# openai/ot-gan

Hardware: AMD Instinct MI355X
Metric: OT-GAN train images/sec (CIFAR-10 32x32, bs=256/GPU) (higher is better)
Workload: dtype f32 (Winograd-domain GEMMs on the fp16 matrix pipe with operands split into two scaled fp16 pieces = 22 significand bits, fp32 accumulate; errors at or below the fp32 MFMA chain's)

## Files before the change

### ot-gan_amd/csrc/winograd.hip

```cpp
#ifndef X3_PIECES
#define X3_PIECES 2
#endif
#ifndef WINO_NS
#define WINO_NS wino_p2
#endif
#include "winograd.h"
#include "gemm_x3.h"
#include <type_traits>

#include <stdlib.h>

#include <algorithm>
#include <array>
#include <atomic>
#include <map>
#include <mutex>
#include <vector>

#include "gemm_tile.h"

namespace WINO_NS {

namespace {

using Cfg = GemmCfg<2, 2, 2, 2, 32>;

template <auto Kern>
inline void ensure_lds(size_t bytes) {
  static const bool done = [bytes] {
    hipFuncSetAttribute(reinterpret_cast<const void*>(Kern), hipFuncAttributeMaxDynamicSharedMemorySize,
                        (int)bytes);
    return true;
  }();
  (void)done;
}


constexpr int WA = kWA;
constexpr int WM = kWA - 2;
constexpr int WF = kWF;
static_assert(WA == 6, "the transforms below are written for F(4x4, 3x3)");

typedef double f64x4 __attribute__((ext_vector_type(4)));

__device__ __forceinline__ f32x4 ld4(const float* p) { return *reinterpret_cast<const f32x4*>(p); }
__device__ __forceinline__ void st4(float* p, f32x4 v) { *reinterpret_cast<f32x4*>(p) = v; }

__device__ __forceinline__ float hdr_scale(const u16* P, int f) {
#if X3_PIECES == 2
  return P ? (reinterpret_cast<const float*>(P) - X3_HDR)[16 + f] : 1.f;
#else
  return 1.f;
#endif
}
__device__ __forceinline__ void st_operand(float* F, u16* P, long rows, int ld, int f, long row, int k, f32x4 v, float sc) {
  if (P) {
    const long fs = op_fstride(rows, ld);
#if X3_PIECES == 2
    st_split4h(P, WF * fs, f * fs + op_off(row, k, ld >> 4), v * sc);
#else
    st_split4(P, WF * fs, f * fs + op_off(row, k, ld >> 4), v);
#endif
  } else {
    st4(F + ((long)f * rows + row) * ld + k, v);
  }
}

__device__ __forceinline__ bool op_thread(bool blocked, long rows, int nk4, long& row, int& k4) {
  if (blocked) {
    const int kgroups = (nk4 + 15) >> 4;
    const long b = blockIdx.x;
    k4 = (int)(b % kgroups) * 16 + (threadIdx.x >> 6) * 4 + (threadIdx.x & 3);
    row = (b / kgroups) * 16 + ((threadIdx.x >> 2) & 15);
  } else {
    const long idx = (long)blockIdx.x * 256 + threadIdx.x;
    k4 = (int)(idx % nk4);
    row = idx / nk4;
  }
  return row < rows && k4 < nk4;
}
inline int op_grid(long rows, long nk4) { return (int)(((rows + 15) / 16) * ((nk4 + 15) / 16)); }

__device__ __forceinline__ void bt1(const f32x4 (&x)[WA], f32x4 (&y)[WA]) {
  y[0] = x[0] - 1.5f * x[1] - 2.f * x[2] + 1.5f * x[3] + x[4];
  y[1] = 0.5f * x[2] - x[1] + 2.5f * x[3] + x[4];
  y[2] = x[1] - 2.5f * x[2] + 0.5f * x[3] + x[4];
  y[3] = 2.f * (x[3] - x[1]) - x[2] + x[4];
  y[4] = 0.5f * (x[1] - x[3]) - x[2] + x[4];
  y[5] = x[1] - 1.5f * x[2] - 2.f * x[3] + 1.5f * x[4] + x[5];
}
template <class V>
__device__ __forceinline__ void at1(const V (&x)[WA], V (&y)[WM]) {
  const V s = x[1] + x[2], d = x[1] - x[2];
  y[0] = x[0] + s + x[3] + x[4];
  y[1] = d + 0.5f * x[3] - 2.f * x[4];
  y[2] = s + 0.25f * x[3] + 4.f * x[4];
  y[3] = d + 0.125f * x[3] - 8.f * x[4] + x[5];
}
__device__ __forceinline__ void a1(const f32x4 (&y)[WM], f32x4 (&x)[WA]) {
  x[0] = y[0];
  x[1] = y[0] + y[1] + y[2] + y[3];
  x[2] = y[0] - y[1] + y[2] - y[3];
  x[3] = y[0] + 0.5f * y[1] + 0.25f * y[2] + 0.125f * y[3];
  x[4] = y[0] - 2.f * y[1] + 4.f * y[2] - 8.f * y[3];
  x[5] = y[3];
}
__device__ __forceinline__ void g1(const f64x4 (&g)[3], f64x4 (&u)[WA]) {
  u[0] = g[0];
  u[1] = (g[0] + g[1] + g[2]) * (1.0 / 3.0);
  u[2] = (g[1] - g[0] - g[2]) * (1.0 / 3.0);
  u[3] = (4.0 * g[0] + 2.0 * g[1] + g[2]) * (-4.0 / 15.0);
  u[4] = (g[0] - 2.0 * g[1] + 4.0 * g[2]) * (1.0 / 15.0);
  u[5] = g[2];
}
__device__ __forceinline__ void gt1(const f32x4 (&u)[WA], f32x4 (&g)[3]) {
  const f32x4 a = u[1] * (1.f / 3.f), b = u[2] * (1.f / 3.f), c = u[3] * (-4.f / 15.f), d = u[4] * (1.f / 15.f);
  g[0] = u[0] + a - b + 4.f * c + d;
  g[1] = a + b + 2.f * c - 2.f * d;
  g[2] = a - b + c + 4.f * d + u[5];
}
__device__ __forceinline__ f64x4 to_d(f32x4 v) { return __builtin_convertvector(v, f64x4); }
__device__ __forceinline__ f32x4 to_f(f64x4 v) { return __builtin_convertvector(v, f32x4); }

template <class Emit>
__device__ __forceinline__ void tf_filter(const f32x4 (&g)[3][3], Emit&& emit) {
  f64x4 t[WA][3];
#pragma unroll
  for (int j = 0; j < 3; ++j) {
    const f64x4 col[3] = {to_d(g[0][j]), to_d(g[1][j]), to_d(g[2][j])};
    f64x4 u[WA];
    g1(col, u);
#pragma unroll
    for (int i = 0; i < WA; ++i) t[i][j] = u[i];
  }
#pragma unroll
  for (int i = 0; i < WA; ++i) {
    f64x4 u[WA];
    g1(t[i], u);
#pragma unroll
    for (int j = 0; j < WA; ++j) emit(i * WA + j, to_f(u[j]));
  }
}
template <class Col>
__device__ __forceinline__ void tf_filter_adj(Col&& col, f32x4 (&dg)[3][3]) {
  f32x4 p[3][WA];
#pragma unroll
  for (int j = 0; j < WA; ++j) {
    f32x4 u[WA], g[3];
    col(j, u);
    gt1(u, g);
#pragma unroll
    for (int i = 0; i < 3; ++i) p[i][j] = g[i];
  }
#pragma unroll
  for (int i = 0; i < 3; ++i) gt1(p[i], dg[i]);
}

struct AmaxArgs {
  const float* x;
  long rows, ld;
  int C;
  float* hdr;
  float gain[WA];
  float fold;
  int floor_one;
  int record_only;
  int nrec;
  float* scratch;
  unsigned* counter;
};
constexpr float kGainBt[WA] = {7.f, 5.f, 5.f, 6.f, 3.f, 7.f};
constexpr float kGainG[WA] = {1.f, 1.f, 1.f, 28.f / 15.f, 7.f / 15.f, 1.f};
constexpr float kGainA[WA] = {1.f, 4.f, 4.f, 1.875f, 15.f, 1.f};
constexpr int kAmaxBlocks = 2048, kAmaxSlots = 64;

__device__ __forceinline__ void write_scales(const AmaxArgs& a, float amax, int tid) {
  if (a.record_only == 2) {
    if (tid == 0) {
      unsigned* p = reinterpret_cast<unsigned*>(a.hdr);
      const unsigned b = __float_as_uint(amax) & 0x7fffffffu;
      if (b > *p) *p = b;
    }
    return;
  }
  if (a.record_only) {
    if (tid < kAmaxSub) a.hdr[tid * kAmaxSubStride] = tid == 0 ? amax : 0.f;
    return;
  }
  if (a.floor_one && amax == amax) amax = fmaxf(amax, 1.f);
  if (tid < WF) {
    const int i = tid / WA, j = tid - i * WA;
    const float bound = amax * a.fold * (a.gain[i] * a.gain[j]);
    float sc = 1.f, inv = 1.f;
    if (!(bound <= 3.0e38f)) {
// ... 57 lines not shown
#pragma unroll
    for (int w = 1; w < 4; ++w) r = (r == r && red[w] == red[w]) ? fmaxf(r, red[w]) : __builtin_nanf("");
    return r;
  };
  m = block_max(m);
  if (tid == 0) {
    __hip_atomic_store(&a.scratch[blockIdx.x], m, __ATOMIC_RELAXED, __HIP_MEMORY_SCOPE_AGENT);
    asm volatile("s_waitcnt vmcnt(0)" ::: "memory");
    last = __hip_atomic_fetch_add(a.counter, 1u, __ATOMIC_RELAXED, __HIP_MEMORY_SCOPE_AGENT) == gridDim.x - 1;
  }
  __syncthreads();
  if (!last) return;
  float r = 0.f;
  for (int i = tid; i < (int)gridDim.x; i += 256) {
    const float w = __hip_atomic_load(&a.scratch[i], __ATOMIC_RELAXED, __HIP_MEMORY_SCOPE_AGENT);
    r = (r == r && w == w) ? fmaxf(r, w) : __builtin_nanf("");
  }
  const float amax = block_max(r);
  write_scales(a, amax, tid);
  if (tid == 0) *a.counter = 0;
}
__global__ __launch_bounds__(64) void scales_from_amax_kernel(AmaxArgs a) { write_scales(a, amax_records_value(a.x, a.nrec), threadIdx.x); }

struct View {
  const float* p;
  long sn, sh, sw;
};
struct WView {
  float* p;
  long sn, sh, sw;
};

struct ScaleSrc {
  const float* rec;
  int nrec;
  float gain[WA];
  float fold;
  int floor_one;
};
__device__ __forceinline__ void producer_scale_table(const ScaleSrc& ss, u16* P, float* s_sc) {
#if X3_PIECES == 2
  if (P) {
    const int tid = threadIdx.x;
    if (tid < WF) {
      float* hdr = reinterpret_cast<float*>(P) - X3_HDR;
      float sc;
      if (ss.rec) {
        float amax = amax_records_value(ss.rec, ss.nrec);
        if (ss.floor_one && amax == amax) amax = fmaxf(amax, 1.f);
        const int i = tid / WA, j = tid - i * WA;
        const float bound = amax * ss.fold * (ss.gain[i] * ss.gain[j]);
        float inv = 1.f;
        sc = 1.f;
        if (!(bound <= 3.0e38f)) {
          sc = inv = __builtin_nanf("");
        } else if (bound > 0.f) {
          const int e = x3_scale_exp(amax * ss.fold, ss.gain[i], ss.gain[j]);
          sc = __builtin_ldexpf(1.f, 14 - e);
          inv = __builtin_ldexpf(1.f, e - 14);
        }
        if (blockIdx.x == 0 && blockIdx.y == 0 && blockIdx.z == 0) {
          hdr[16 + tid] = sc;
          hdr[64 + tid] = inv;
          if (tid == 0) hdr[0] = amax;
        }
      } else {
        sc = hdr[16 + tid];
      }
      s_sc[tid] = sc;
    }
    __syncthreads();
  }
#endif
}
struct InArgs {
  ScaleSrc ss;
  View v[4];
  int coff[4];
  int H, W, TH, TW, C;
  long T;
  int ldv;
  float* V;
  int s2_skip;
  u16* P;
  int up;
  int Cpad;
};
template <int ACT>
__device__ __forceinline__ f32x4 wino_act(f32x4 v) {
#pragma unroll
  for (int j = 0; j < 4; ++j) {
    if (ACT == 1) v[j] = fmaxf(v[j], 0.f);
    if (ACT == 2) v[j] = v[j] > 0.f ? v[j] : expm1f(v[j]);
  }
  return v;
}
template <int ACT, bool DOUBLED>
__global__ __launch_bounds__(256) void wino_input_kernel(InArgs a) {
  __shared__ float s_sc[WF];
  producer_scale_table(a.ss, a.P, s_sc);
  long t;
  int k4;
  if (!op_thread(a.P != nullptr, a.T, (a.Cpad > a.C ? a.Cpad : a.C) >> 2, t, k4)) return;
  const int c = k4 * 4;
  const int tb = (int)(t % a.TW), ta = (int)((t / a.TW) % a.TH);
  const long n = t / ((long)a.TW * a.TH);
  const int cls = blockIdx.z;
  const View v = a.v[cls];
  const int pass = DOUBLED ? (int)blockIdx.y : 0;
  const f32x4 zero = {0.f, 0.f, 0.f, 0.f};
  if (c >= a.C) {
    for (int f = 0; f < WF; ++f) st_operand(a.V, a.P, a.T, a.ldv, f, t, c, zero, 1.f);
    return;
  }
  f32x4 T[WA][WA];
#pragma unroll
  for (int j = 0; j < WA; ++j) {
    const int q = WM * tb - 1 + j;
    f32x4 col[WA], o[WA];
#pragma unroll
    for (int i = 0; i < WA; ++i) {
      const int r = WM * ta - 1 + i;
      const bool ok = (unsigned)r < (unsigned)a.H && (unsigned)q < (unsigned)a.W;
      f32x4 e = ok ? ld4(v.p + n * v.sn + (r >> a.up) * v.sh + (q >> a.up) * v.sw + c) : zero;
      if (ACT != 0 || DOUBLED) e = wino_act<ACT>(pass ? -e : e);
      col[i] = e;
    }
    bt1(col, o);
#pragma unroll
    for (int i = 0; i < WA; ++i) T[i][j] = o[i];
  }
  const int k0 = a.coff[cls] + c + (pass ? a.C : 0);
#pragma unroll
  for (int i = 0; i < WA; ++i) {
    f32x4 o[WA];
    bt1(T[i], o);
#pragma unroll
    for (int j = 0; j < WA; ++j)
      if (a.s2_skip < 0 || s2_present(cls, i * WA + j, a.s2_skip)) st_operand(a.V, a.P, a.T, a.ldv, i * WA + j, t, k0, o[j], s_sc[i * WA + j]);
  }
}

struct OutArgs {
  WView v[4];
  int coff[4];
  int TH, TW, C;
  long T;
  int ldm;
  const float* Mh;
  const float* bias;
  int accumulate;
  float* amax;
  WView gv[4];
};
__global__ __launch_bounds__(256) void wino_output_kernel(OutArgs a) {
  const int c4n = a.C >> 2;
  const long idx = (long)blockIdx.x * 256 + threadIdx.x;
  if (idx >= a.T * c4n) return;
  unsigned mb = 0u;
  const int c = (int)(idx % c4n) * 4;
  const long t = idx / c4n;
  const int tb = (int)(t % a.TW), ta = (int)((t / a.TW) % a.TH);
  const long n = t / ((long)a.TW * a.TH);
  const WView v = a.v[blockIdx.z];
  const float* in = a.Mh + t * a.ldm + a.coff[blockIdx.z] + c;
  const long fs = a.T * a.ldm;
  f32x4 S[WM][WA];
#pragma unroll
  for (int j = 0; j < WA; ++j) {
    f32x4 col[WA], o[WM];
#pragma unroll
    for (int i = 0; i < WA; ++i) col[i] = ld4(in + (i * WA + j) * fs);
    at1(col, o);
#pragma unroll
    for (int i = 0; i < WM; ++i) S[i][j] = o[i];
  }
  f32x4 b = {0.f, 0.f, 0.f, 0.f};
  if (a.bias) b = ld4(a.bias + c);
#pragma unroll
  for (int i = 0; i < WM; ++i) {
    f32x4 y[WM];
    at1(S[i], y);
#pragma unroll
    for (int j = 0; j < WM; ++j) {
      float* dst = v.p + n * v.sn + (WM * ta + i) * v.sh + (WM * tb + j) * v.sw + c;
      f32x4 o = y[j] + b;
      if (a.accumulate) o += ld4(dst);
      mb = amax_bits4(o, mb);
      st4(dst, o);
    }
  }
  if (a.amax) amax_commit(a.amax, mb);
}

__device__ __forceinline__ float wino_sigmoid(float x) { return 1.f / (1.f + expf(-x)); }
__global__ __launch_bounds__(256) void wino_output_glu_kernel(OutArgs a) {
  const int ch = a.C >> 1, c4n = ch >> 2;
  const long idx = (long)blockIdx.x * 256 + threadIdx.x;
  if (idx >= a.T * c4n) return;
  unsigned mb = 0u;
  const int c = (int)(idx % c4n) * 4;
  const long t = idx / c4n;
  const int tb = (int)(t % a.TW), ta = (int)((t / a.TW) % a.TH);
  const long n = t / ((long)a.TW * a.TH);
  const WView v = a.v[blockIdx.z], gv = a.gv[blockIdx.z];
  const long fs = a.T * a.ldm;
#pragma unroll
  for (int half = 0; half < 2; ++half) {
    const int cc = c + half * ch;
    const float* in = a.Mh + t * a.ldm + a.coff[blockIdx.z] + cc;
    f32x4 S[WM][WA];
#pragma unroll
    for (int j = 0; j < WA; ++j) {
      f32x4 col[WA], o[WM];
#pragma unroll
      for (int i = 0; i < WA; ++i) col[i] = ld4(in + (i * WA + j) * fs);
      at1(col, o);
#pragma unroll
      for (int i = 0; i < WM; ++i) S[i][j] = o[i];
    }
    f32x4 b = {0.f, 0.f, 0.f, 0.f};
    if (a.bias) b = ld4(a.bias + cc);
#pragma unroll
    for (int i = 0; i < WM; ++i) {
      f32x4 y[WM];
      at1(S[i], y);
#pragma unroll
      for (int j = 0; j < WM; ++j) {
        float* dst = v.p + n * v.sn + (WM * ta + i) * v.sh + (WM * tb + j) * v.sw + c;
        const f32x4 o = y[j] + b;
        st4(dst + half * ch, o);
        if (half) {
          const f32x4 val = ld4(dst);
          f32x4 gl;
#pragma unroll
          for (int k = 0; k < 4; ++k) gl[k] = val[k] * wino_sigmoid(o[k]);
          mb = amax_bits4(gl, mb);
          st4(gv.p + n * gv.sn + (WM * ta + i) * gv.sh + (WM * tb + j) * gv.sw + c, gl);
        }
      }
    }
  }
  if (a.amax) amax_commit(a.amax, mb);
}

__global__ __launch_bounds__(256) void op_zero_cols_kernel(u16* P, long rows, int ld, int k0, int k1) {
  long row;
  int k4;
  if (!op_thread(true, rows, (k1 - k0) >> 2, row, k4)) return;
  const f32x4 z = {0.f, 0.f, 0.f, 0.f};
  for (int f = 0; f < WF; ++f) st_operand(nullptr, P, rows, ld, f, row, k0 + 4 * k4, z, 1.f);
}

__global__ __launch_bounds__(256) void wino_outadj_kernel(InArgs a) {
  __shared__ float s_sc[WF];
  producer_scale_table(a.ss, a.P, s_sc);
  long t;
  int k4;
  if (!op_thread(a.P != nullptr, a.T, a.C >> 2, t, k4)) return;
  const int c = k4 * 4;
  const int tb = (int)(t % a.TW), ta = (int)((t / a.TW) % a.TH);
  const long n = t / ((long)a.TW * a.TH);
  const View v = a.v[blockIdx.z];
  f32x4 u[WA][WM];
#pragma unroll
  for (int j = 0; j < WM; ++j) {
    f32x4 col[WM], o[WA];
#pragma unroll
    for (int i = 0; i < WM; ++i) col[i] = ld4(v.p + n * v.sn + (WM * ta + i) * v.sh + (WM * tb + j) * v.sw + c);
    a1(col, o);
#pragma unroll
    for (int i = 0; i < WA; ++i) u[i][j] = o[i];
  }
#pragma unroll
  for (int i = 0; i < WA; ++i) {
    f32x4 o[WA];
    a1(u[i], o);
#pragma unroll
    for (int j = 0; j < WA; ++j) st_operand(a.V, a.P, a.T, a.ldv, i * WA + j, t, a.coff[blockIdx.z] + c, o[j], s_sc[i * WA + j]);
  }
}

__global__ __launch_bounds__(256) void wino_filter_fwd_kernel(const float* __restrict__ weffT, long cls_stride,
                                                            int Cin, int Cout, float* __restrict__ U, u16* P) {
  const long rows = 4L * Cout;
  long row;
  int k4;
  if (!op_thread(P != nullptr, rows, Cin >> 2, row, k4)) return;
  const int ci = k4 * 4;
  const int cls = (int)(row / Cout), co = (int)(row % Cout);
  const float* src = weffT + cls * cls_stride + (long)co * 9 * Cin + ci;
  f32x4 g[3][3];
#pragma unroll
  for (int i = 0; i < 3; ++i)
#pragma unroll
    for (int j = 0; j < 3; ++j) g[i][j] = ld4(src + (long)(i * 3 + j) * Cin);
  tf_filter(g, [&](int f, f32x4 v) { st_operand(U, P, rows, Cin, f, row, ci, v, hdr_scale(P, f)); });
}

__global__ __launch_bounds__(256) void wino_filter_bwd_kernel(const float* __restrict__ weff, long cls_stride,
                                                            int Cin, int Cout, float* __restrict__ U, u16* P) {
  const int c4n = Cout >> 2;
  long row;
  int k4;
  if (!op_thread(P != nullptr, Cin, 4 * c4n, row, k4)) return;
  const int ci = (int)row, cls = k4 / c4n, co = (k4 % c4n) * 4;
  const float* src = weff + cls * cls_stride + (long)ci * Cout + co;
  f32x4 g[3][3];
#pragma unroll
  for (int i = 0; i < 3; ++i)
#pragma unroll
    for (int j = 0; j < 3; ++j) g[i][j] = ld4(src + (long)((2 - i) * 3 + (2 - j)) * Cin * Cout);
  tf_filter(g, [&](int f, f32x4 v) { st_operand(U, P, Cin, 4 * Cout, f, ci, cls * Cout + co, v, hdr_scale(P, f)); });
}

__device__ __forceinline__ int fold5_tap(int p, int k) { return p ? (k + 1) >> 1 : k >> 1; }

__global__ __launch_bounds__(256) void wino_filter_fwd_unfolded_kernel(const float* __restrict__ wT, int Cin, int Cout,
                                                                     float* __restrict__ U, u16* P) {
  const long rows = 4L * Cout;
  long row;
  int k4;
  if (!op_thread(P != nullptr, rows, Cin >> 2, row, k4)) return;
  const int ci = k4 * 4;
  const int cls = (int)(row / Cout), co = (int)(row % Cout);
  const int ph = cls >> 1, pw = cls & 1;
  const float* src = wT + (long)co * 25 * Cin + ci;
  const f32x4 zero = {0.f, 0.f, 0.f, 0.f};
  f32x4 g[3][3];
#pragma unroll
  for (int i = 0; i < 3; ++i)
#pragma unroll
    for (int j = 0; j < 3; ++j) g[i][j] = zero;
#pragma unroll
  for (int kh = 0; kh < 5; ++kh)
#pragma unroll
    for (int kw = 0; kw < 5; ++kw) {
      const f32x4 v = ld4(src + (long)(kh * 5 + kw) * Cin);
#pragma unroll
      for (int i = 0; i < 3; ++i)
#pragma unroll
        for (int j = 0; j < 3; ++j)
          if (fold5_tap(ph, kh) == i && fold5_tap(pw, kw) == j) g[i][j] += v;
    }
  tf_filter(g, [&](int f, f32x4 v) { st_operand(U, P, rows, Cin, f, row, ci, v, hdr_scale(P, f)); });
}

__global__ __launch_bounds__(256) void wino_filter_bwd_unfolded_kernel(const float* __restrict__ w, int Cin, int Cout,
                                                                     float* __restrict__ U, u16* P) {
  const int c4n = Cout >> 2;
  long row;
  int k4;
  if (!op_thread(P != nullptr, Cin, 4 * c4n, row, k4)) return;
  const int ci = (int)row, cls = k4 / c4n, co = (k4 % c4n) * 4;
  const int ph = cls >> 1, pw = cls & 1;
  const float* src = w + (long)ci * Cout + co;
  const f32x4 zero = {0.f, 0.f, 0.f, 0.f};
  f32x4 g[3][3];
#pragma unroll
  for (int i = 0; i < 3; ++i)
#pragma unroll
    for (int j = 0; j < 3; ++j) g[i][j] = zero;
#pragma unroll
  for (int kh = 0; kh < 5; ++kh)
#pragma unroll
    for (int kw = 0; kw < 5; ++kw) {
      const f32x4 v = ld4(src + (long)(kh * 5 + kw) * Cin * Cout);
#pragma unroll
      for (int i = 0; i < 3; ++i)
#pragma unroll
        for (int j = 0; j < 3; ++j)
          if (fold5_tap(ph, kh) == 2 - i && fold5_tap(pw, kw) == 2 - j) g[i][j] += v;
    }
  tf_filter(g, [&](int f, f32x4 v) { st_operand(U, P, Cin, 4 * Cout, f, ci, cls * Cout + co, v, hdr_scale(P, f)); });
}

__device__ __forceinline__ f32x4 wn_mul4(f32x4 v, f32x4 sc) {
#pragma clang fp contract(off)
  return v * sc;
}
__device__ __forceinline__ f32x4 wn_gather4(const float* __restrict__ p, long stride, float sc) {
  const f32x4 v = {p[0], p[stride], p[2 * stride], p[3 * stride]};
  const f32x4 s = {sc, sc, sc, sc};
  return wn_mul4(v, s);
}
__device__ __forceinline__ bool raw_wave(long rows, int ngroups, int quads, long& row0, int& group, int& sub) {
  const int per = (ngroups + quads - 1) / quads, halves = blockDim.x >> 8;
  const int wave = threadIdx.x >> 6;
  sub = wave & 3;
  group = (int)(blockIdx.x % per) * quads + (quads == 4 ? sub : 0);
  row0 = (long)(blockIdx.x / per) * (16 * halves) + (wave >> 2) * 16;
  return row0 < rows && group < ngroups;
}
__device__ __forceinline__ f32x4 raw_to_store_lane(f32x4 v) {
  const int lane = threadIdx.x & 63, src = (lane & 3) * 16 + ((lane >> 2) & 15);
  f32x4 r;
#pragma unroll
  for (int k = 0; k < 4; ++k) r[k] = __int_as_float(__builtin_amdgcn_ds_bpermute(src << 2, __float_as_int(v[k])));
  return r;
}
constexpr int kRawMinWorkgroups = 512;
inline int raw_halves(long rows, int ngroups, int quads) {
  return ((rows + 31) / 32) * ((ngroups + quads - 1) / quads) >= kRawMinWorkgroups ? 2 : 1;
}
inline int raw_grid(long rows, int ngroups, int quads, int halves) {
  return (int)(((rows + 16 * halves - 1) / (16 * halves)) * ((ngroups + quads - 1) / quads));
}

__global__ __launch_bounds__(512) void wino_filter_fwd_raw_kernel(const float* __restrict__ V, const float* __restrict__ scale,
                                                                int Cin, int Cout, float* __restrict__ U, u16* P) {
  long co0;
  int grp, cls;
  if (!raw_wave(Cout, Cin >> 4, 1, co0, grp, cls)) return;
  const int lane = threadIdx.x & 63;
  const int ph = cls >> 1, pw = cls & 1;
  f32x4 g[3][3];
  {
    long co = co0 + (lane & 15);
    if (co >= Cout) co = Cout - 1;
    const float* src = V + (long)(grp * 16 + (lane >> 4) * 4) * Cout + co;
    const float sc = scale[co];
    const f32x4 zero = {0.f, 0.f, 0.f, 0.f};
#pragma unroll
    for (int i = 0; i < 3; ++i)
#pragma unroll
      for (int j = 0; j < 3; ++j) g[i][j] = zero;
#pragma unroll
    for (int kh = 0; kh < 5; ++kh)
#pragma unroll
      for (int kw = 0; kw < 5; ++kw) {
        const f32x4 v = wn_gather4(src + (long)(kh * 5 + kw) * Cin * Cout, Cout, sc);
#pragma unroll
        for (int i = 0; i < 3; ++i)
#pragma unroll
          for (int j = 0; j < 3; ++j)
            if (fold5_tap(ph, kh) == i && fold5_tap(pw, kw) == j) g[i][j] += v;
      }
  }
#pragma unroll
  for (int i = 0; i < 3; ++i)
#pragma unroll
    for (int j = 0; j < 3; ++j) g[i][j] = raw_to_store_lane(g[i][j]);
  const long co = co0 + ((lane >> 2) & 15);
  if (co >= Cout) return;
  const int ci = grp * 16 + (lane & 3) * 4;
  const long rows = 4L * Cout, row = cls * (long)Cout + co;
  tf_filter(g, [&](int f, f32x4 v) { st_operand(U, P, rows, Cin, f, row, ci, v, hdr_scale(P, f)); });
}

__global__ __launch_bounds__(256) void wino_filter_bwd_raw_kernel(const float* __restrict__ V, const float* __restrict__ scale,
                                                                int Cin, int Cout, float* __restrict__ U, u16* P) {
  const int c4n = Cout >> 2;
  long row;
  int k4;
  if (!op_thread(P != nullptr, Cin, 4 * c4n, row, k4)) return;
  const int ci = (int)row, cls = k4 / c4n, co = (k4 % c4n) * 4;
  const int ph = cls >> 1, pw = cls & 1;
  const float* src = V + (long)ci * Cout + co;
  const f32x4 sc = ld4(scale + co);
  const f32x4 zero = {0.f, 0.f, 0.f, 0.f};
  f32x4 g[3][3];
#pragma unroll
  for (int i = 0; i < 3; ++i)
#pragma unroll
    for (int j = 0; j < 3; ++j) g[i][j] = zero;
#pragma unroll
  for (int kh = 0; kh < 5; ++kh)
#pragma unroll
    for (int kw = 0; kw < 5; ++kw) {
      const f32x4 v = wn_mul4(ld4(src + (long)(kh * 5 + kw) * Cin * Cout), sc);
#pragma unroll
      for (int i = 0; i < 3; ++i)
#pragma unroll
        for (int j = 0; j < 3; ++j)
          if (fold5_tap(ph, kh) == 2 - i && fold5_tap(pw, kw) == 2 - j) g[i][j] += v;
    }
  tf_filter(g, [&](int f, f32x4 v) { st_operand(U, P, Cin, 4 * Cout, f, ci, cls * Cout + co, v, hdr_scale(P, f)); });
}

__global__ __launch_bounds__(256) void wino_filter_adj_kernel(const float* __restrict__ slabs, int nsplit,
                                                            long split_stride, int Cin, int Cout,
                                                            float* __restrict__ dweff, long cls_stride) {
  const int c4n = Cout >> 2;
  const long idx = (long)blockIdx.x * 256 + threadIdx.x;
  if (idx >= 4L * Cin * c4n) return;
  const int co = (int)(idx % c4n) * 4;
  const long r = idx / c4n;
  const int ci = (int)(r % Cin), cls = (int)(r / Cin);
  const long ldu = 4L * Cout, fs = (long)Cin * ldu;
  const float* src = slabs + (long)ci * ldu + (long)cls * Cout + co;
  f32x4 dg[3][3];
  tf_filter_adj(
      [&](int j, f32x4(&u)[WA]) {
#pragma unroll
        for (int i = 0; i < WA; ++i) {
          f32x4 s = ld4(src + (i * WA + j) * fs);
          for (int k = 1; k < nsplit; ++k) s += ld4(src + k * split_stride + (i * WA + j) * fs);
          u[i] = s;
        }
      },
      dg);
  float* dst = dweff + cls * cls_stride + (long)ci * Cout + co;
#pragma unroll
  for (int i = 0; i < 3; ++i)
#pragma unroll
    for (int j = 0; j < 3; ++j) st4(dst + (long)(i * 3 + j) * Cin * Cout, dg[i][j]);
}


__device__ __forceinline__ float quad_lane(float v, int lane_in_quad) {
  const int x = __float_as_int(v);
  int r;
  switch (lane_in_quad) {
    case 0: r = __builtin_amdgcn_update_dpp(0, x, 0x00, 0xF, 0xF, true); break;
    case 1: r = __builtin_amdgcn_update_dpp(0, x, 0x55, 0xF, 0xF, true); break;
    case 2: r = __builtin_amdgcn_update_dpp(0, x, 0xAA, 0xF, 0xF, true); break;
    default: r = __builtin_amdgcn_update_dpp(0, x, 0xFF, 0xF, 0xF, true); break;
  }
  return __int_as_float(r);
}
__global__ __launch_bounds__(256) void wino_filter_adj_unfold5_kernel(const float* __restrict__ slabs, int nsplit,
                                                                    long split_stride, int Cin, int Cout,
                                                                    float* __restrict__ dw) {
  const int c4n = Cout >> 2;
  const long idx = (long)blockIdx.x * 64 + (threadIdx.x >> 2);
  const int cls = threadIdx.x & 3;
  if (idx >= (long)Cin * c4n) return;
  const int co = (int)(idx % c4n) * 4;
  const int ci = (int)(idx / c4n);
  const long ldu = 4L * Cout, fs = (long)Cin * ldu;
  const float* src = slabs + (long)ci * ldu + (long)cls * Cout + co;
  f32x4 dg[3][3];
  tf_filter_adj(
      [&](int j, f32x4(&u)[WA]) {
#pragma unroll
        for (int i = 0; i < WA; ++i) {
          f32x4 sv = ld4(src + (i * WA + j) * fs);
          for (int k = 1; k < nsplit; ++k) sv += ld4(src + k * split_stride + (i * WA + j) * fs);
          u[i] = sv;
        }
      },
      dg);
  constexpr int TH[2][5] = {{0, 0, 1, 1, 2}, {0, 1, 1, 2, 2}};
  const bool ph = (cls >> 1) != 0, pw = (cls & 1) != 0;
  float* dst = dw + (long)ci * Cout + co;
#pragma unroll
  for (int kh = 0; kh < 5; ++kh) {
    f32x4 row[3];
#pragma unroll
    for (int j = 0; j < 3; ++j)
#pragma unroll
      for (int c = 0; c < 4; ++c) row[j][c] = ph ? dg[TH[1][kh]][j][c] : dg[TH[0][kh]][j][c];
#pragma unroll
    for (int kw = 0; kw < 5; ++kw) {
      f32x4 sum;
#pragma unroll
      for (int c = 0; c < 4; ++c) {
        const float x = pw ? row[TH[1][kw]][c] : row[TH[0][kw]][c];
        float acc = 0.f + quad_lane(x, 0);
        acc += quad_lane(x, 1);
        acc += quad_lane(x, 2);
        acc += quad_lane(x, 3);
        sum[c] = acc;
      }
      if (((kh * 5 + kw) & 3) == cls) st4(dst + (long)(kh * 5 + kw) * Cin * Cout, sum);
    }
  }
}

__device__ __forceinline__ int s2_tap(int parity, int i) {
  return parity ? 2 * i : (i == 0 ? -1 : 2 * i - 1);
}

__global__ __launch_bounds__(256) void wino_s2_filter_fwd_kernel(const float* __restrict__ wT, int Ceff, int Cout,
                                                               float* __restrict__ U, u16* P, int plain, int ld) {
  const int c4n = Ceff >> 2, ncls = plain ? 1 : 4, kk = plain ? 3 : 5;
  long row;
  int k4;
  if (!op_thread(P != nullptr, Cout, ncls * c4n, row, k4)) return;
  const int co = (int)row, cls = k4 / c4n, ce = (k4 % c4n) * 4;
  const int pi = cls >> 1, pj = cls & 1;
  const f32x4 zero = {0.f, 0.f, 0.f, 0.f};
  f32x4 g[3][3];
#pragma unroll
  for (int i = 0; i < 3; ++i)
#pragma unroll
    for (int j = 0; j < 3; ++j) {
      const int kh = plain ? i : s2_tap(pi, i), kw = plain ? j : s2_tap(pj, j);
      g[i][j] = (kh >= 0 && kw >= 0) ? ld4(wT + ((long)co * kk * kk + kh * kk + kw) * Ceff + ce) : zero;
    }
  tf_filter(g, [&](int f, f32x4 v) {
    if (plain || s2_present(cls, f, 0))
      st_operand(U, P, Cout, ld, f, co, cls * Ceff + ce, v, hdr_scale(P, f));
  });
}

__global__ __launch_bounds__(256) void wino_s2_filter_bwd_kernel(const float* __restrict__ w, int Ceff, int Cout,
                                                               float* __restrict__ U, u16* P, int plain, int Kp) {
  long r;
  int k4;
// ... 509 lines not shown
}

int x3_wgrad_splits(int M, int N, long T) {
  const int blocks = ((M + X3_BM - 1) / X3_BM) * ((N + X3_BN - 1) / X3_BN) * WF;
  constexpr int target = 256;
  int ns = (target + blocks - 1) / blocks;
  if (ns > 16) ns = 16;
  const int nkt = (int)((T + X3_BK - 1) / X3_BK);
  while (ns > 1 && nkt / ns < 8) --ns;
  return ns < 1 ? 1 : ns;
}

int wgrad_splits(const WinoGeo& g) {
  const long T = wino_tiles(g);
  const int blocks = ((g.Cin + 127) / 128) * ((4 * g.Cout + 127) / 128) * WF;
  int ns = (1024 + blocks - 1) / blocks;
  if (ns > 8) ns = 8;
  const int nkt = (int)((T + Cfg::BK - 1) / Cfg::BK);
  while (ns > 1 && nkt / ns < 8) --ns;
  return ns < 1 ? 1 : ns;
}

}

void producer_scales(InArgs& ia, const float* x, long rows, int C, long ld, float* base, const float (&gain)[WA], float fold,
                     bool floor_one, hipStream_t s, const float* given, int given_count = 1) {
  ia.ss.rec = nullptr;
  ia.ss.nrec = 1;
  if (X3_NP != 2) return;
  if (given) {
    ia.ss.rec = given;
    ia.ss.nrec = given_count > 1 ? given_count : 1;
    for (int i = 0; i < WA; ++i) ia.ss.gain[i] = gain[i];
    ia.ss.fold = fold;
    ia.ss.floor_one = floor_one ? 1 : 0;
    return;
  }
  op_scales(x, rows, C, ld, base, gain, fold, floor_one, s, given, false, false, given_count);
}
void wino_absmax(const float* x, long rows, int C, long ld, float* record, hipStream_t s, bool accumulate) {
  const float unit[WA] = {1.f, 1.f, 1.f, 1.f, 1.f, 1.f};
  op_scales(x, rows, C, ld, record, unit, 1.f, false, s, nullptr, true, accumulate);
}

bool winograd_enabled() {
  static const bool on = [] {
    const char* e = getenv("OTGAN_DISABLE_WINOGRAD");
    return !(e && e[0] == '1');
  }();
  return on;
}

size_t wino_x_operand_floats(const WinoGeo& g) {
  const long T = wino_tiles(g);
  const bool ok = use_x3() && g.Cin % X3_BK == 0 && use_x3_wgrad_tl() && T % 32 == 0 && (4 * g.Cout) % 32 == 0;
  return ok ? operand_floats(op_elems(T, g.Cin)) : 0;
}

size_t wino_fwd_ws_floats(const WinoGeo& g) {
  const size_t T = (size_t)wino_tiles(g);
  return operand_floats(op_elems(T, g.Cin)) + operand_floats(op_elems(T, 4 * g.Cout)) +
         operand_floats(std::max(op_elems(4 * g.Cout, g.Cin), op_elems(g.Cin, 4 * g.Cout))) +
         WF * T * (size_t)(4 * g.Cout > g.Cin ? 4 * g.Cout : g.Cin);
}
size_t wino_dgrad_ws_floats(const WinoGeo& g) { return wino_fwd_ws_floats(g); }
size_t wino_wgrad_ws_floats(const WinoGeo& g) {
  const size_t T = (size_t)wino_tiles(g);
  const size_t Tp = (T + 63) / 64 * 64;
  const int ns = std::max(wgrad_splits(g), x3_wgrad_splits(g.Cin, 4 * g.Cout, (long)Tp));
  return operand_floats(std::max(op_elems(g.Cin, Tp), op_elems(Tp, g.Cin))) +
         operand_floats(std::max(op_elems(4 * g.Cout, Tp), op_elems(Tp, 4 * g.Cout))) + (size_t)ns * WF * 4 * g.Cout * g.Cin;
}

size_t wino_filter_floats(const WinoGeo& g, int which) {
  return (which == 0 || which == 2) ? operand_floats(op_elems(4 * g.Cout, g.Cin)) : operand_floats(op_elems(g.Cin, 4 * g.Cout));
}
int wino_prepare_filters(const WinoGeo& g, int which, const float* w, long cls_stride, float* out, hipStream_t s) {
  const int N4 = 4 * g.Cout;
  if (which == 2) {
    const bool x3 = use_x3() && g.Cin % X3_BK == 0;
    if (x3) op_scales(w, 1, 25 * g.Cin * g.Cout, 0, out, kGainG, 4.f, false, s, g.w_amax);
    hipLaunchKernelGGL(wino_filter_fwd_unfolded_kernel, dim3(op_grid(N4, g.Cin / 4)), dim3(256), 0, s, w, g.Cin, g.Cout, out,
                       x3 ? op_planes(out) : nullptr);
    return OTGAN_OK;
  }
  if (which == 3) {
    const bool x3 = use_x3() && N4 % X3_BK == 0;
    if (x3) op_scales(w, 1, 25 * g.Cin * g.Cout, 0, out, kGainG, 4.f, false, s, g.w_amax);
    hipLaunchKernelGGL(wino_filter_bwd_unfolded_kernel, dim3(op_grid(g.Cin, g.Cout)), dim3(256), 0, s, w, g.Cin, g.Cout, out,
                       x3 ? op_planes(out) : nullptr);
    return OTGAN_OK;
  }
  if (which == 0) {
    const bool x3 = use_x3() && g.Cin % X3_BK == 0;
    if (x3) op_scales(w, 4, 9 * g.Cin * g.Cout, cls_stride, out, kGainG, 1.f, false, s);
    hipLaunchKernelGGL(wino_filter_fwd_kernel, dim3(op_grid(N4, g.Cin / 4)), dim3(256), 0, s, w, cls_stride, g.Cin,
                       g.Cout, out, x3 ? op_planes(out) : nullptr);
  } else {
    const bool x3 = use_x3() && N4 % X3_BK == 0;
    if (x3) op_scales(w, 4, 9 * g.Cin * g.Cout, cls_stride, out, kGainG, 1.f, false, s);
    hipLaunchKernelGGL(wino_filter_bwd_kernel, dim3(op_grid(g.Cin, g.Cout)), dim3(256), 0, s, w, cls_stride, g.Cin,
                       g.Cout, out, x3 ? op_planes(out) : nullptr);
  }
  return OTGAN_OK;
}

int wino_prepare_filters_raw(const WinoGeo& g, int which, const float* V, const float* scale, float* out, hipStream_t s) {
  const int N4 = 4 * g.Cout;
  if (which == 2) {
    const bool x3 = use_x3() && g.Cin % X3_BK == 0;
    if (x3) op_scales(V, 1, 25 * g.Cin * g.Cout, 0, out, kGainG, 4.f, false, s, g.w_amax);
    const int hv = raw_halves(g.Cout, g.Cin / 16, 1);
    hipLaunchKernelGGL(wino_filter_fwd_raw_kernel, dim3(raw_grid(g.Cout, g.Cin / 16, 1, hv)), dim3(256 * hv), 0, s, V, scale,
                       g.Cin, g.Cout, out, x3 ? op_planes(out) : nullptr);
  } else {
    const bool x3 = use_x3() && N4 % X3_BK == 0;
    if (x3) op_scales(V, 1, 25 * g.Cin * g.Cout, 0, out, kGainG, 4.f, false, s, g.w_amax);
    hipLaunchKernelGGL(wino_filter_bwd_raw_kernel, dim3(op_grid(g.Cin, g.Cout)), dim3(256), 0, s, V, scale, g.Cin, g.Cout,
                       out, x3 ? op_planes(out) : nullptr);
  }
  return OTGAN_OK;
}

int wino_fwd(const WinoGeo& g, const float* x, const float* weffT, long cls_stride, const float* bias, float* y,
             float* ws, hipStream_t s, const float* prep) {
  const long T = wino_tiles(g);
  const int N4 = 4 * g.Cout;
  const bool x3 = use_x3() && g.Cin % X3_BK == 0;
  const size_t nV = op_elems(T, g.Cin), nU = op_elems(N4, g.Cin);
  float* V = (g.x_op && x3) ? g.x_op : ws;
  float* Uws = ws + operand_floats(nV);
  float* Mh = Uws + operand_floats(nU);
  float* U = prep ? const_cast<float*>(prep) : Uws;
  u16* VP = x3 ? op_planes(V) : nullptr;
  u16* UP = x3 ? op_planes(U) : nullptr;
  if (!prep) wino_prepare_filters(g, 0, weffT, cls_stride, U, s);
  InArgs ia;
  memset(&ia, 0, sizeof(ia));
  ia.s2_skip = -1;
  ia.v[0].p = x; ia.v[0].sn = (long)g.H * g.W * g.ldx; ia.v[0].sh = (long)g.W * g.ldx; ia.v[0].sw = g.ldx;
  ia.H = g.H; ia.W = g.W; ia.TH = g.H / WM; ia.TW = g.W / WM; ia.C = g.Cin; ia.T = T; ia.ldv = g.Cin; ia.V = V;
  ia.P = VP;
  if (x3) producer_scales(ia, x, (long)g.N * g.H * g.W, g.Cin, g.ldx, V, kGainBt, 1.f, false, s, g.x_amax);
  hipLaunchKernelGGL((wino_input_kernel<0, false>), dim3(op_grid(T, g.Cin / 4), 1, 1), dim3(256), 0, s, ia);
  BgArgs b;
  memset(&b, 0, sizeof(b));
  b.Ap = VP; b.Bp = UP; b.pA = (long)nV; b.pB = (long)nU;
  if (x3) { b.hdrA = op_hdr(V); b.hdrB = op_hdr(U); }
  b.A = V; b.B = U; b.C = Mh; b.M = (int)T; b.N = N4; b.K = g.Cin;
  b.lda = g.Cin; b.ldb = g.Cin; b.ldc = N4;
  b.sA = T * g.Cin; b.sB = (long)N4 * g.Cin; b.sC = T * N4;
  b.tiles_m = (int)((T + Cfg::BM - 1) / Cfg::BM); b.tiles_n = (N4 + Cfg::BN - 1) / Cfg::BN;
  b.kt_per_split = (g.Cin + Cfg::BK - 1) / Cfg::BK;
  launch_bgemm<false>(b, 1, s);
  OutArgs oa;
  memset(&oa, 0, sizeof(oa));
  class_views(g, y + g.y_coff, g.ldy, oa.v);
  for (int cls = 0; cls < 4; ++cls) oa.coff[cls] = cls * g.Cout;
  oa.TH = g.H / WM; oa.TW = g.W / WM; oa.C = g.Cout; oa.T = T; oa.ldm = N4; oa.Mh = Mh; oa.bias = bias;
  if (g.glu_out) {
    class_views(g, g.glu_out, g.Cout / 2, oa.gv);
    oa.amax = g.glu_amax;
    hipLaunchKernelGGL(wino_output_glu_kernel, dim3(grid1(T * (g.Cout / 8)), 1, 4), dim3(256), 0, s, oa);
    return OTGAN_OK;
  }
  hipLaunchKernelGGL(wino_output_kernel, dim3(grid1(T * (g.Cout / 4)), 1, 4), dim3(256), 0, s, oa);
  return OTGAN_OK;
}

int wino_dgrad(const WinoGeo& g, const float* dy, const float* weff, long cls_stride, float* dx, int lddx,
               int accumulate, float* ws, hipStream_t s, const float* prep) {
  const long T = wino_tiles(g);
  const int K4 = 4 * g.Cout;
  const bool x3 = use_x3() && K4 % X3_BK == 0;
  const size_t nV = op_elems(T, K4), nU = op_elems(g.Cin, K4);
  float* DV = ws;
  float* Uws = DV + operand_floats(nV);
  float* Xh = Uws + operand_floats(nU);
  float* U = prep ? const_cast<float*>(prep) : Uws;
  u16* VP = x3 ? op_planes(DV) : nullptr;
  u16* UP = x3 ? op_planes(U) : nullptr;
  if (!prep) wino_prepare_filters(g, 1, weff, cls_stride, U, s);
  InArgs ia;
  memset(&ia, 0, sizeof(ia));
  ia.s2_skip = -1;
  class_views(g, dy + g.y_coff, g.ldy, ia.v);
  for (int cls = 0; cls < 4; ++cls) ia.coff[cls] = cls * g.Cout;
  ia.H = g.H; ia.W = g.W; ia.TH = g.H / WM; ia.TW = g.W / WM; ia.C = g.Cout; ia.T = T; ia.ldv = K4; ia.V = DV;
  ia.P = VP;
  if (x3) producer_scales(ia, dy + g.y_coff, (long)g.N * 4 * g.H * g.W, g.Cout, g.ldy, DV, kGainBt, 1.f, false, s, g.dy_amax);
  hipLaunchKernelGGL((wino_input_kernel<0, false>), dim3(op_grid(T, g.Cout / 4), 1, 4), dim3(256), 0, s, ia);
  BgArgs b;
  memset(&b, 0, sizeof(b));
  b.Ap = VP; b.Bp = UP; b.pA = (long)nV; b.pB = (long)nU;
  if (x3) { b.hdrA = op_hdr(DV); b.hdrB = op_hdr(U); }
  b.A = DV; b.B = U; b.C = Xh; b.M = (int)T; b.N = g.Cin; b.K = K4;
  b.lda = K4; b.ldb = K4; b.ldc = g.Cin;
  b.sA = T * K4; b.sB = (long)g.Cin * K4; b.sC = T * g.Cin;
  b.tiles_m = (int)((T + Cfg::BM - 1) / Cfg::BM); b.tiles_n = (g.Cin + Cfg::BN - 1) / Cfg::BN;
  b.kt_per_split = (K4 + Cfg::BK - 1) / Cfg::BK;
  launch_bgemm<false>(b, 1, s);
  OutArgs oa;
  memset(&oa, 0, sizeof(oa));
  oa.v[0].p = dx; oa.v[0].sn = (long)g.H * g.W * lddx; oa.v[0].sh = (long)g.W * lddx; oa.v[0].sw = lddx;
  oa.TH = g.H / WM; oa.TW = g.W / WM; oa.C = g.Cin; oa.T = T; oa.ldm = g.Cin; oa.Mh = Xh; oa.bias = nullptr;
  oa.accumulate = accumulate;
  hipLaunchKernelGGL(wino_output_kernel, dim3(grid1(T * (g.Cin / 4)), 1, 1), dim3(256), 0, s, oa);
  return OTGAN_OK;
}

int wino_wgrad(const WinoGeo& g, const float* x, const float* dy, float* dweff, long cls_stride, float* ws,
               hipStream_t s, float* dw_unfolded5) {
  const long T = wino_tiles(g);
  const int N4 = 4 * g.Cout;
  if (use_x3_wgrad_tl() && T % 32 == 0 && g.Cin % 32 == 0 && N4 % 32 == 0) {
    const int ns = x3_wgrad_splits(g.Cin, N4, T);
    const size_t nV = op_elems(T, g.Cin), nM = op_elems(T, N4);
    float* Vb = g.x_op ? g.x_op : ws;
    u16* VP = op_planes(Vb);
    float* Mb = ws + operand_floats(nV);
    u16* MP = op_planes(Mb);
    float* slabs = ws + operand_floats(nV) + operand_floats(nM);
    if (!g.x_op) {
      InArgs ia;
      memset(&ia, 0, sizeof(ia));
      ia.s2_skip = -1;
      ia.v[0].p = x; ia.v[0].sn = (long)g.H * g.W * g.ldx; ia.v[0].sh = (long)g.W * g.ldx; ia.v[0].sw = g.ldx;
      ia.H = g.H; ia.W = g.W; ia.TH = g.H / WM; ia.TW = g.W / WM; ia.C = g.Cin; ia.T = T; ia.ldv = g.Cin; ia.P = VP;
      producer_scales(ia, x, (long)g.N * g.H * g.W, g.Cin, g.ldx, Vb, kGainBt, 1.f, false, s, g.x_amax);
      hipLaunchKernelGGL((wino_input_kernel<0, false>), dim3(op_grid(T, g.Cin / 4), 1, 1), dim3(256), 0, s, ia);
    }
    InArgs da;
    memset(&da, 0, sizeof(da));
    da.s2_skip = -1;
    class_views(g, dy + g.y_coff, g.ldy, da.v);
    for (int cls = 0; cls < 4; ++cls) da.coff[cls] = cls * g.Cout;
    da.H = g.H; da.W = g.W; da.TH = g.H / WM; da.TW = g.W / WM; da.C = g.Cout; da.T = T; da.ldv = N4; da.P = MP;
    producer_scales(da, dy + g.y_coff, (long)g.N * 4 * g.H * g.W, g.Cout, g.ldy, Mb, kGainA, 1.f, false, s, g.dy_amax);
    hipLaunchKernelGGL(wino_outadj_kernel, dim3(op_grid(T, g.Cout / 4), 1, 4), dim3(256), 0, s, da);
    BgArgs b;
    memset(&b, 0, sizeof(b));
    b.Ap = VP; b.Bp = MP; b.hdrA = op_hdr(Vb); b.hdrB = op_hdr(Mb);
    b.C = slabs; b.M = g.Cin; b.N = N4; b.K = (int)T;
    b.ldc = N4; b.sC = (long)g.Cin * N4; b.sSplit = (long)WF * g.Cin * N4;
    b.kt_per_split = (int)((T / X3_BK + ns - 1) / ns);
    launch_bgemm_tl(b, ns, s);
    if (dw_unfolded5)
      hipLaunchKernelGGL(wino_filter_adj_unfold5_kernel, dim3(grid1(4L * g.Cin * (g.Cout / 4))), dim3(256), 0, s, slabs, ns,
                         (long)WF * g.Cin * N4, g.Cin, g.Cout, dw_unfolded5);
    else
      hipLaunchKernelGGL(wino_filter_adj_kernel, dim3(grid1(4L * g.Cin * (g.Cout / 4))), dim3(256), 0, s, slabs, ns,
                         (long)WF * g.Cin * N4, g.Cin, g.Cout, dweff, cls_stride);
    return OTGAN_OK;
  }
  const int ns = wgrad_splits(g);
  const size_t nV = WF * (size_t)T * g.Cin, nM = WF * (size_t)T * N4;
  float* V = ws;
  float* dM = V + operand_floats(nV);
  float* slabs = dM + operand_floats(nM);
  InArgs ia;
  memset(&ia, 0, sizeof(ia));
  ia.s2_skip = -1;
  ia.v[0].p = x; ia.v[0].sn = (long)g.H * g.W * g.ldx; ia.v[0].sh = (long)g.W * g.ldx; ia.v[0].sw = g.ldx;
  ia.H = g.H; ia.W = g.W; ia.TH = g.H / WM; ia.TW = g.W / WM; ia.C = g.Cin; ia.T = T; ia.ldv = g.Cin; ia.V = V;
  hipLaunchKernelGGL((wino_input_kernel<0, false>), dim3(op_grid(T, g.Cin / 4), 1, 1), dim3(256), 0, s, ia);
  InArgs da;
  memset(&da, 0, sizeof(da));
  da.s2_skip = -1;
  class_views(g, dy + g.y_coff, g.ldy, da.v);
  for (int cls = 0; cls < 4; ++cls) da.coff[cls] = cls * g.Cout;
  da.H = g.H; da.W = g.W; da.TH = g.H / WM; da.TW = g.W / WM; da.C = g.Cout; da.T = T; da.ldv = N4; da.V = dM;
  hipLaunchKernelGGL(wino_outadj_kernel, dim3(op_grid(T, g.Cout / 4), 1, 4), dim3(256), 0, s, da);
  BgArgs b;
  memset(&b, 0, sizeof(b));
  b.A = V; b.B = dM; b.C = slabs; b.M = g.Cin; b.N = N4; b.K = (int)T;
  b.lda = g.Cin; b.ldb = N4; b.ldc = N4;
  b.sA = T * g.Cin; b.sB = T * N4; b.sC = (long)g.Cin * N4; b.sSplit = (long)WF * g.Cin * N4;
  b.tiles_m = (g.Cin + Cfg::BM - 1) / Cfg::BM; b.tiles_n = (N4 + Cfg::BN - 1) / Cfg::BN;
  const int nkt = (int)((T + Cfg::BK - 1) / Cfg::BK);
  b.kt_per_split = (nkt + ns - 1) / ns;
  launch_bgemm<true>(b, ns, s);
  if (dw_unfolded5)
    hipLaunchKernelGGL(wino_filter_adj_unfold5_kernel, dim3(grid1(4L * g.Cin * (g.Cout / 4))), dim3(256), 0, s, slabs, ns,
                       (long)WF * g.Cin * N4, g.Cin, g.Cout, dw_unfolded5);
  else
    hipLaunchKernelGGL(wino_filter_adj_kernel, dim3(grid1(4L * g.Cin * (g.Cout / 4))), dim3(256), 0, s, slabs, ns,
                       (long)WF * g.Cin * N4, g.Cin, g.Cout, dweff, cls_stride);
  return OTGAN_OK;
}

namespace {

template <class V, class P>
void parity_views(int H, int W, P base, int ld, V (&v)[4]) {
  for (int cls = 0; cls < 4; ++cls) {
    const int pi = cls >> 1, pj = cls & 1;
    v[cls].p = base + ((long)pi * W + pj) * ld;
    v[cls].sn = (long)H * W * ld;
    v[cls].sh = 2L * W * ld;
    v[cls].sw = 2L * ld;
  }
}

template <class V, class P>
void s2_views(const WinoS2Geo& g, P base, int ld, V (&v)[4]) {
  if (!g.plain) return parity_views(g.H, g.W, base, ld, v);
  v[0].p = base;
  v[0].sn = (long)g.H * g.W * ld;
  v[0].sh = (long)g.W * ld;
// ... 340 lines not shown
```

Before: 30740.

## Share identical Winograd filter rows across up5 phase classes and skip duplicate GEMM segments

For the folded 5x5 upsampling conv, several Winograd-domain filter entries are identical across the four phase classes, so only the owning class writes them. The batched GEMM is told to skip the duplicate segments (seg_mode/seg_skip), and the output transform reads the shared entries from the owner class's column offset. This removes redundant GEMM work and filter stores. It adds per-element offset logic in the output kernels, and it is correct only if the ownership pattern matches the GEMM skip logic. The sharing is enabled unconditionally in the forward path, which may be wrong for geometries that are not up5.

```diff
diff --git a/ot-gan_amd/csrc/winograd.hip b/ot-gan_amd/csrc/winograd.hip
--- a/ot-gan_amd/csrc/winograd.hip
+++ b/ot-gan_amd/csrc/winograd.hip
@@ -40,6 +40,9 @@
 constexpr int WM = kWA - 2;
 constexpr int WF = kWF;
 static_assert(WA == 6, "the transforms below are written for F(4x4, 3x3)");
+
+constexpr int kUp5Shared = 1;
+__host__ __device__ __forceinline__ bool up5_owner(int cls, int f) { return s2_present(cls, f, kUp5Shared); }
 
 typedef double f64x4 __attribute__((ext_vector_type(4)));
 
@@ -403,7 +406,21 @@
   int accumulate;
   float* amax;
   WView gv[4];
+  int up5_shared;
 };
+struct OutShare {
+  int row1, col1, both;
+  __device__ __forceinline__ int at(int i, int j) const { return i == 1 ? (j == 1 ? both : row1) : (j == 1 ? col1 : 0); }
+};
+__device__ __forceinline__ OutShare out_share(const OutArgs& a, int cls) {
+  OutShare s = {0, 0, 0};
+  if (a.up5_shared) {
+    s.row1 = a.coff[cls | 2] - a.coff[cls];
+    s.col1 = a.coff[cls | 1] - a.coff[cls];
+    s.both = a.coff[3] - a.coff[cls];
+  }
+  return s;
+}
 __global__ __launch_bounds__(256) void wino_output_kernel(OutArgs a) {
   const int c4n = a.C >> 2;
   const long idx = (long)blockIdx.x * 256 + threadIdx.x;
@@ -415,13 +432,14 @@
   const long n = t / ((long)a.TW * a.TH);
   const WView v = a.v[blockIdx.z];
   const float* in = a.Mh + t * a.ldm + a.coff[blockIdx.z] + c;
+  const OutShare sh = out_share(a, blockIdx.z);
   const long fs = a.T * a.ldm;
   f32x4 S[WM][WA];
 #pragma unroll
   for (int j = 0; j < WA; ++j) {
     f32x4 col[WA], o[WM];
 #pragma unroll
-    for (int i = 0; i < WA; ++i) col[i] = ld4(in + (i * WA + j) * fs);
+    for (int i = 0; i < WA; ++i) col[i] = ld4(in + sh.at(i, j) + (i * WA + j) * fs);
     at1(col, o);
 #pragma unroll
     for (int i = 0; i < WM; ++i) S[i][j] = o[i];
@@ -456,6 +474,7 @@
   const long n = t / ((long)a.TW * a.TH);
   const WView v = a.v[blockIdx.z], gv = a.gv[blockIdx.z];
   const long fs = a.T * a.ldm;
+  const OutShare sh = out_share(a, blockIdx.z);
 #pragma unroll
   for (int half = 0; half < 2; ++half) {
     const int cc = c + half * ch;
@@ -465,7 +484,7 @@
     for (int j = 0; j < WA; ++j) {
       f32x4 col[WA], o[WM];
 #pragma unroll
-      for (int i = 0; i < WA; ++i) col[i] = ld4(in + (i * WA + j) * fs);
+      for (int i = 0; i < WA; ++i) col[i] = ld4(in + sh.at(i, j) + (i * WA + j) * fs);
       at1(col, o);
 #pragma unroll
       for (int i = 0; i < WM; ++i) S[i][j] = o[i];
@@ -546,7 +565,9 @@
   for (int i = 0; i < 3; ++i)
 #pragma unroll
     for (int j = 0; j < 3; ++j) g[i][j] = ld4(src + (long)(i * 3 + j) * Cin);
-  tf_filter(g, [&](int f, f32x4 v) { st_operand(U, P, rows, Cin, f, row, ci, v, hdr_scale(P, f)); });
+  tf_filter(g, [&](int f, f32x4 v) {
+    if (up5_owner(cls, f)) st_operand(U, P, rows, Cin, f, row, ci, v, hdr_scale(P, f));
+  });
 }
 
 __global__ __launch_bounds__(256) void wino_filter_bwd_kernel(const float* __restrict__ weff, long cls_stride,
@@ -594,7 +615,9 @@
         for (int j = 0; j < 3; ++j)
           if (fold5_tap(ph, kh) == i && fold5_tap(pw, kw) == j) g[i][j] += v;
     }
-  tf_filter(g, [&](int f, f32x4 v) { st_operand(U, P, rows, Cin, f, row, ci, v, hdr_scale(P, f)); });
+  tf_filter(g, [&](int f, f32x4 v) {
+    if (up5_owner(cls, f)) st_operand(U, P, rows, Cin, f, row, ci, v, hdr_scale(P, f));
+  });
 }
 
 __global__ __launch_bounds__(256) void wino_filter_bwd_unfolded_kernel(const float* __restrict__ w, int Cin, int Cout,
@@ -696,7 +719,9 @@
   if (co >= Cout) return;
   const int ci = grp * 16 + (lane & 3) * 4;
   const long rows = 4L * Cout, row = cls * (long)Cout + co;
-  tf_filter(g, [&](int f, f32x4 v) { st_operand(U, P, rows, Cin, f, row, ci, v, hdr_scale(P, f)); });
+  tf_filter(g, [&](int f, f32x4 v) {
+    if (up5_owner(cls, f)) st_operand(U, P, rows, Cin, f, row, ci, v, hdr_scale(P, f));
+  });
 }
 
 __global__ __launch_bounds__(256) void wino_filter_bwd_raw_kernel(const float* __restrict__ V, const float* __restrict__ scale,
@@ -1512,9 +1537,11 @@
   b.sA = T * g.Cin; b.sB = (long)N4 * g.Cin; b.sC = T * N4;
   b.tiles_m = (int)((T + Cfg::BM - 1) / Cfg::BM); b.tiles_n = (N4 + Cfg::BN - 1) / Cfg::BN;
   b.kt_per_split = (g.Cin + Cfg::BK - 1) / Cfg::BK;
+  b.seg_mode = 2; b.seg_len = g.Cout; b.seg_skip = kUp5Shared;
   launch_bgemm<false>(b, 1, s);
   OutArgs oa;
   memset(&oa, 0, sizeof(oa));
+  oa.up5_shared = 1;
   class_views(g, y + g.y_coff, g.ldy, oa.v);
   for (int cls = 0; cls < 4; ++cls) oa.coff[cls] = cls * g.Cout;
   oa.TH = g.H / WM; oa.TW = g.W / WM; oa.C = g.Cout; oa.T = T; oa.ldm = N4; oa.Mh = Mh; oa.bias = bias;
```

Result: no change. 31040, median of 6 (+1.0%).
